# kestrelquantum/QuantumCollocation.jl

Hardware: AMD Instinct MI355X
Metric: full-trajectory constraint+Jacobian evals/s, 3-qubit T=1000 (higher is better)
Workload: dtype f64; 1 GPU; 3-qubit Toffoli UnitarySmoothPulseProblem, T=1000; T=1000 knots (1000/GPU), Pade order 4, free dt; T=1000, N=8, n_drives=6, kernel=mfma, parallelism=knot-shard x1, output_ring_buffers=17

## Files before the change

quantumcollocation.jl_amd/csrc/qc_mfma_exp.hip:

```cpp
#include <stdlib.h>

#include "qc_mfma_common.h"

namespace {

using namespace qc_mfma;

constexpr int kXDeg = 8;
constexpr double kXTh = 0.125;
constexpr int kXMmax = 8;

__device__ inline v4d ximg(const double* __restrict__ Gx, int mat, int lane) {
    const v2d* p = reinterpret_cast<const v2d*>(Gx) + mat * 128 + lane;
    const v2d lo = p[0], hi = p[64];
    return v4d{lo[0], lo[1], hi[0], hi[1]};
}
template <int CTRL>
__device__ inline double xdpp(double x) {
    int lo = __double2loint(x), hi = __double2hiint(x);
    lo = __builtin_amdgcn_update_dpp(0, lo, CTRL, 0xf, 0xf, false);
    hi = __builtin_amdgcn_update_dpp(0, hi, CTRL, 0xf, 0xf, false);
    return __hiloint2double(hi, lo);
}
__device__ inline double xreadlane(double x, int l) {
    return __hiloint2double(__builtin_amdgcn_readlane(__double2hiint(x), l), __builtin_amdgcn_readlane(__double2loint(x), l));
}

template <int M, bool JAC>
__device__ __forceinline__ void horner_step(const v4d& Y, const v4d (&Gj)[M], v4d& R, v4d (&Q)[M], const v4d& cI) {
    v4d accR = cI;
    v4d acc[M];
    const v4d z = {0.0, 0.0, 0.0, 0.0};
    accR = __builtin_amdgcn_mfma_f64_16x16x4f64(Y[0], R[0], accR, 0, 0, 0);
    if constexpr (JAC) {
#pragma unroll
        for (int q = 0; q < M; ++q) acc[q] = __builtin_amdgcn_mfma_f64_16x16x4f64(Gj[q][0], R[0], z, 0, 0, 0);
    }
#pragma unroll
    for (int kk = 1; kk < 4; ++kk) {
        accR = __builtin_amdgcn_mfma_f64_16x16x4f64(Y[kk], R[kk], accR, 0, 0, 0);
        if constexpr (JAC) {
#pragma unroll
            for (int q = 0; q < M; ++q) acc[q] = __builtin_amdgcn_mfma_f64_16x16x4f64(Gj[q][kk], R[kk], acc[q], 0, 0, 0);
        }
    }
    if constexpr (JAC) {
#pragma unroll
        for (int kk = 0; kk < 4; ++kk) {
#pragma unroll
            for (int q = 0; q < M; ++q) acc[q] = __builtin_amdgcn_mfma_f64_16x16x4f64(Y[kk], Q[q][kk], acc[q], 0, 0, 0);
        }
#pragma unroll
        for (int q = 0; q < M; ++q) Q[q] = acc[q];
    }
    R = accR;
}

template <int M>
__device__ __forceinline__ void horner_step_ell(const v4d& Y, const double (&tw)[M][4], const int (&tc)[M][4], double* __restrict__ scr, v4d& R,
                                                v4d (&Q)[M], const v4d& cI, int g, int j) {
#pragma unroll
    for (int r = 0; r < 4; ++r) scr[(4 * r + g) * 17 + j] = R[r];
    __builtin_amdgcn_fence(__ATOMIC_RELEASE, "wavefront");
    __builtin_amdgcn_wave_barrier();
    __builtin_amdgcn_fence(__ATOMIC_ACQUIRE, "wavefront");
    double x[M][4];
#pragma unroll
    for (int q = 0; q < M; ++q) {
#pragma unroll
        for (int r = 0; r < 4; ++r) x[q][r] = scr[tc[q][r]];
    }
    __builtin_amdgcn_sched_barrier(0);
    const v4d z = {0.0, 0.0, 0.0, 0.0};
    v4d accR = cI, acc[M];
#pragma unroll
    for (int kk = 0; kk < 4; ++kk) {
        accR = __builtin_amdgcn_mfma_f64_16x16x4f64(Y[kk], R[kk], accR, 0, 0, 0);
#pragma unroll
        for (int q = 0; q < M; ++q) acc[q] = __builtin_amdgcn_mfma_f64_16x16x4f64(Y[kk], Q[q][kk], kk == 0 ? z : acc[q], 0, 0, 0);
    }
#pragma unroll
    for (int q = 0; q < M; ++q) {
#pragma unroll
        for (int r = 0; r < 4; ++r) Q[q][r] = __builtin_fma(tw[q][r], x[q][r], acc[q][r]);
    }
    R = accR;
    __builtin_amdgcn_fence(__ATOMIC_RELEASE, "wavefront");
    __builtin_amdgcn_wave_barrier();
    __builtin_amdgcn_fence(__ATOMIC_ACQUIRE, "wavefront");
}

template <int M, bool JAC>
__device__ __forceinline__ void square_step(const v4d& Et, const v4d (&Kt)[M], v4d& E, v4d (&L)[M]) {
    const v4d z = {0.0, 0.0, 0.0, 0.0};
    v4d accE = z, acc[M];
#pragma unroll
    for (int kk = 0; kk < 4; ++kk) {
        accE = __builtin_amdgcn_mfma_f64_16x16x4f64(Et[kk], E[kk], accE, 0, 0, 0);
        if constexpr (JAC) {
#pragma unroll
            for (int q = 0; q < M; ++q) acc[q] = __builtin_amdgcn_mfma_f64_16x16x4f64(Et[kk], L[q][kk], kk == 0 ? z : acc[q], 0, 0, 0);
        }
    }
    if constexpr (JAC) {
#pragma unroll
        for (int kk = 0; kk < 4; ++kk) {
#pragma unroll
            for (int q = 0; q < M; ++q) acc[q] = __builtin_amdgcn_mfma_f64_16x16x4f64(Kt[q][kk], E[kk], acc[q], 0, 0, 0);
        }
#pragma unroll
        for (int q = 0; q < M; ++q) L[q] = acc[q];
    }
    E = accE;
}

template <bool JAC, int kMU, int kW, bool ELL = false, int kIPW = 1>
__global__ __launch_bounds__(64 * kW * kIPW, kW) void qc_mfma16_exp_kernel(const QcParams P, const double* __restrict__ Z, double* __restrict__ F,
                                                                    double* __restrict__ J) {
    qc_kernarg_touch<sizeof(QcParams) + 64>();
    static_assert(kIPW == 1 || kW == 2, "two intervals per workgroup: the two-wave forms");
    __shared__ double scr_all[kIPW * kW * (kMU + 1) * 16 * 17];
    const int lane = threadIdx.x & 63;
    const int wq = kIPW * kW > 1 ? __builtin_amdgcn_readfirstlane(threadIdx.x >> 6) : 0;
    const int wv = kW > 1 ? wq % kW : 0;
    double* __restrict__ scr = scr_all + wq * ((kMU + 1) * 16 * 17);
    const int d0 = wv * kMU;
    const int m = P.m;
    const int g = lane >> 4, j = lane & 15, jj = j & 7;
    const bool ft = P.off_dt >= 0;
    const double* __restrict__ Gx = P.Gx;
    const v4d IdB = identity_B(g, j);
    const v4d zero = {0.0, 0.0, 0.0, 0.0};

    {
        const int b = qc_xcd_remap((int)blockIdx.x, (P.n_int + kIPW - 1) / kIPW) * kIPW + wq / kW;
        if (b >= P.n_int) return;
        const long long t = P.t_begin + b;
        const double* __restrict__ z0 = Z + t * (long long)P.zdim;
        const double* __restrict__ z1 = z0 + P.zdim;
        double* __restrict__ Jb = JAC ? J + (size_t)b * P.J_stride + P.J_off : nullptr;
        double* __restrict__ Fb = F ? F + (size_t)b * P.F_stride + P.F_off : nullptr;
        const double h = ft ? z0[P.off_dt] : opaque_scalar(P.dt_fixed);

        const int nc = P.nc, jc = jj < nc ? jj : 0, nr = P.n;
        v4d u0, u1;
#pragma unroll
        for (int r = 0; r < 4; ++r) {
            const int row = 4 * r + g;
            u0[r] = row < nr ? z0[P.off_U + jc * nr + row] : 0.0;
            u1[r] = row < nr ? z1[P.off_U + jc * nr + row] : 0.0;
        }
        v4d Gj[kMU];
        double tw[kMU][4];
        int tc[kMU][4];
        v4d Ga = ximg(Gx, 0, lane);
        {
            constexpr int kMA = kXMmax;
            v4d img[kMA];
            double ak[kMA];
#pragma unroll
            for (int u = 0; u < kMA; ++u) {
                const int k = u < m ? u : (m > 0 ? m - 1 : 0);
                img[u] = ximg(Gx, m > 0 ? k + 1 : 0, lane);
                ak[u] = (u < m) ? z0[P.off_a + k] : 0.0;
            }
            if constexpr (ELL) {
                const double* __restrict__ bw = reinterpret_cast<const double*>(P.ell16);
                const int* __restrict__ bc = reinterpret_cast<const int*>(reinterpret_cast<const char*>(P.ell16) + kXMmax * 32 * 8);
#pragma unroll
                for (int u = 0; u < kMU; ++u) {
#pragma unroll
                    for (int r = 0; r < 4; ++r) {
                        tw[u][r] = bw[(d0 + u) * 32 + 4 * r + g];
                        tc[u][r] = bc[(d0 + u) * 32 + 4 * r + g] * 17 + j;
                    }
                }
            } else {
#pragma unroll
                for (int u = 0; u < kMU; ++u) {
                    const int k = d0 + u;
                    Gj[u] = ximg(Gx, k < m ? k + 1 : 0, lane);
                }
            }
#pragma unroll
            for (int u = 0; u < kMA; ++u) Ga += ak[u] * img[u];
        }
        if constexpr (!ELL) {
#pragma unroll
            for (int u = 0; u < kMU; ++u) if (d0 + u >= m) Gj[u] = zero;
        }

        int sq = 0;
        {
            double best = 0.0;
            bool bad = false;
#pragma unroll
            for (int kk = 0; kk < 4; ++kk) {
                double c = fabs(h * Ga[kk]);
                c += xdpp<0x128>(c);
                c += xdpp<0x124>(c);
                c += xdpp<0x122>(c);
                c += xdpp<0x121>(c);
#pragma unroll
                for (int r = 0; r < 4; ++r) {
                    const double v = xreadlane(c, 16 * r);
                    if (!(v == v) || v > 1e300) bad = true;
                    best = fmax(best, v);
                }
            }
            if (!bad && best > kXTh) {
                int e;
                (void)frexp(best / kXTh, &e);
                sq = e;
                if (ldexp(kXTh, e - 1) >= best) sq = e - 1;
                sq = sq < 0 ? 0 : (sq > 60 ? 60 : sq);
            }
        }
        const double sc = ldexp(1.0, -sq);
        const v4d Y = (h * sc) * Ga;

        double fact = 1.0;
#pragma unroll
        for (int k = 2; k <= kXDeg; ++k) fact *= (double)k;
        double ck = 1.0 / fact;
        v4d R = ck * IdB;
        v4d Q[kMU];
#pragma unroll
        for (int u = 0; u < kMU; ++u) Q[u] = zero;
#pragma unroll 1
        for (int k = kXDeg; k >= 1; --k) {
            ck *= (double)k;
            if constexpr (ELL) horner_step_ell<kMU>(Y, tw, tc, scr, R, Q, ck * IdB, g, j);
            else horner_step<kMU, JAC>(Y, Gj, R, Q, ck * IdB);
        }
        for (int q = 0; q < sq; ++q) {
            v4d Et, Kt[kMU];
            if constexpr (JAC) {
                v4d in[kMU + 1], out[kMU + 1];
                in[0] = R;
#pragma unroll
                for (int u = 0; u < kMU; ++u) in[u + 1] = Q[u];
                lds_transpose16_multi<kMU + 1>(scr, in, out, g, j);
                Et = out[0];
#pragma unroll
                for (int u = 0; u < kMU; ++u) Kt[u] = out[u + 1];
            } else {
                Et = lds_transpose16(scr, R, g, j);
            }
            square_step<kMU, JAC>(Et, Kt, R, Q);
        }
        const v4d Et = lds_transpose16(scr, R, g, j);
        const v4d EU = mm16(Et, u0);
        if (Fb && wv == 0) {
            const v4d dT = lds_transpose16(scr, u1 - EU, g, j);
#pragma unroll
            for (int r = 0; r < 2; ++r) if (4 * r + g < nc && j < nr) qc_st8m<2>(Fb + (4 * r + g) * nr + j, dT[r]);
        }
        if constexpr (JAC) {
            double* pF = Jb + P.jo_F;
            const v4d mE = -Et;
#pragma unroll
            for (int q = wv * (8 / kW); q < (wv + 1) * (8 / kW); ++q) {
                if (q < nc) {
#pragma unroll
                    for (int r = 0; r < 4; ++r) if (4 * r + g < nr && j < nr) qc_st8m<2>(pF + q * nr * nr + (4 * r + g) * nr + j, mE[r]);
                }
            }
            if (wv == kW - 1) for (int i = lane; i < P.s; i += 64) Jb[P.jo_B + i] = 1.0;
            const double fac = -(h * sc);
            v4d Kt[kMU], XT[kMU], ua[kMU];
            lds_transpose16_multi<kMU>(scr, Q, Kt, g, j);
#pragma unroll
            for (int u = 0; u < kMU; ++u) ua[u] = u0;
            mm16_multi<kMU>(ua, Kt, XT);
#pragma unroll
            for (int u = 0; u < kMU; ++u) {
                if (d0 + u < m) {
#pragma unroll
                    for (int r = 0; r < 2; ++r)
                        if (4 * r + g < nc && j < nr) qc_st8m<2>(Jb + P.jo_a + (size_t)(d0 + u) * P.s + (4 * r + g) * nr + j, fac * XT[u][r]);
                }
            }
            if (ft && wv == 0) {
                const v4d GEU = mm16(Ga, EU);
                const v4d hT = lds_transpose16(scr, -GEU, g, j);
#pragma unroll
                for (int r = 0; r < 2; ++r) if (4 * r + g < nc && j < nr) qc_st8m<2>(Jb + P.jo_h + (4 * r + g) * nr + j, hT[r]);
            }
        }
        if (wv == kW - 1) deriv_rows_generic(P, z0, z1, h, Fb, Jb, lane, false);
    }
}

}

bool qc_mfma_exp_supported(const QcParams& P) {
    return P.integrator == QC_EXPONENTIAL && P.n <= 16 && P.nc <= 8 && P.m <= kXMmax;
}

hipError_t qc_launch_mfma_exp(const QcParams& P, bool ell, const double* dZ, double* dF, double* dJ, hipStream_t st) {
    const int grid = P.n_int;
#define QC_XJ1(MU_, W_, I_) do { const int wgs = (grid + I_ - 1) / I_; \
                            if (ell) hipLaunchKernelGGL((qc_mfma16_exp_kernel<true, MU_, W_, true, I_>), dim3(wgs), dim3(64 * W_ * I_), 0, st, P, dZ, dF, dJ); \
                            else hipLaunchKernelGGL((qc_mfma16_exp_kernel<true, MU_, W_, false, I_>), dim3(wgs), dim3(64 * W_ * I_), 0, st, P, dZ, dF, dJ); } while (0)
#define QC_XJ(MU_, W_) do { if (W_ == 2 && grid > 256) QC_XJ1(MU_, W_, (W_ == 2 ? 2 : 1)); else QC_XJ1(MU_, W_, 1); } while (0)
    if (!dJ) {
        hipLaunchKernelGGL((qc_mfma16_exp_kernel<false, 1, 1>), dim3(grid), dim3(64), 0, st, P, dZ, dF, dJ);
    } else if (P.m <= 1) {
        QC_XJ(1, 1);
    } else if (!ell && P.n_int >= 768) {
        if (P.m <= 2) hipLaunchKernelGGL((qc_mfma16_exp_kernel<true, 2, 1>), dim3(grid), dim3(64), 0, st, P, dZ, dF, dJ);
        else if (P.m <= 4) hipLaunchKernelGGL((qc_mfma16_exp_kernel<true, 4, 1>), dim3(grid), dim3(64), 0, st, P, dZ, dF, dJ);
        else if (P.m <= 6) hipLaunchKernelGGL((qc_mfma16_exp_kernel<true, 6, 1>), dim3(grid), dim3(64), 0, st, P, dZ, dF, dJ);
        else hipLaunchKernelGGL((qc_mfma16_exp_kernel<true, 8, 1>), dim3(grid), dim3(64), 0, st, P, dZ, dF, dJ);
    } else {
        const int mh = (P.m + 1) / 2;
        if (mh == 1) QC_XJ(1, 2);
        else if (mh == 2) QC_XJ(2, 2);
        else if (mh == 3) QC_XJ(3, 2);
        else QC_XJ(4, 2);
    }
#undef QC_XJ
#undef QC_XJ1
    return hipGetLastError();
}
```

Measured before the change: 125,000 evals/s (T=1000-equivalent).

## Replace degree-8 Horner Taylor exp with degree-12 Paterson-Stockmeyer evaluation

Replaces the degree-8 Horner Taylor evaluation of the matrix exponential (threshold 1/8) with a degree-12 Taylor polynomial evaluated Paterson–Stockmeyer style from powers A, A², A³, A⁴ plus two outer products, with the scaling threshold raised to 1/2. The aim is fewer MFMA products per interval, both from fewer squarings and from fewer polynomial steps, including the Fréchet-derivative (Jacobian) chains. To do this it parks intermediate sums in extra LDS, adds transposes, and lowers occupancy for kMU>=4 through the launch bounds. That adds LDS pressure and register use, and the larger threshold may change accuracy. Profiling and validation scripts are added alongside.

```diff
diff --git a/profiles/exp_mfma_model.py b/profiles/exp_mfma_model.py
--- /dev/null
+++ b/profiles/exp_mfma_model.py
@@ -0,0 +1,35 @@
+#!/usr/bin/env python3
+import collections
+import math
+import os
+import sys
+
+import numpy as np
+
+sys.path.insert(0, os.path.dirname(os.path.dirname(os.path.abspath(__file__))))
+import __graft_entry__ as g
+
+
+def squarings(norm, th):
+    if not norm > th:
+        return 0
+    e = math.frexp(norm / th)[1]
+    return e - 1 if math.ldexp(th, e - 1) >= norm else e
+
+
+qc = g.load_package()
+inp = qc.config_inputs(3, T=1000, integrator="exponential")
+tr, sys_ = inp.traj, inp.integrators[0].system
+Z = tr.datavec.reshape(tr.T, -1)
+m = sys_.n_drives
+G0, Gd = np.array(sys_.G_drift), np.array(sys_.G_drives).reshape(m, 16, 16)
+a, dt = Z[:, tr.offset("a"):tr.offset("a") + m], Z[:, tr.offset("Δt")]
+norms = [np.abs(dt[t] * (G0 + np.tensordot(a[t], Gd, 1))).sum(axis=0).max() for t in range(tr.T - 1)]
+kW, kMU = 2, 3
+gather, product = 4 + 4 * kMU, 4 + 8 * kMU
+outputs = kW * (4 + 4 * kMU) + 4
+for name, th, fixed in (("degree 8, Horner, threshold 1/8", 0.125, 8 * gather), ("degree 12 in five products, threshold 1/2", 0.5, 3 * gather + 2 * product)):
+    sq = [squarings(x, th) for x in norms]
+    jac = sum(kW * (fixed + s * product) + outputs for s in sq)
+    res = sum((8 if th == 0.125 else 5) * 4 + 4 * s + 4 for s in sq)
+    print(f"{name}: squarings {dict(sorted(collections.Counter(sq).items()))}; F + dF {jac} MFMAs a launch ({jac / len(sq):.1f} an interval), F alone {res}")
diff --git a/profiles/exp_outputs.py b/profiles/exp_outputs.py
--- /dev/null
+++ b/profiles/exp_outputs.py
@@ -0,0 +1,34 @@
+#!/usr/bin/env python3
+import os
+import sys
+
+import numpy as np
+
+ROOT = os.path.dirname(os.path.dirname(os.path.abspath(__file__)))
+sys.path.insert(0, ROOT)
+sys.path.insert(0, os.path.join(ROOT, "tests"))
+
+
+def rel(a, b):
+    return float(np.max(np.abs(a - b) / np.maximum(np.abs(b), 1e-300), initial=0.0, where=b != 0))
+
+
+if sys.argv[1] == "dump":
+    import __graft_entry__ as g
+    import oracle.qc_oracle_c as oc
+    from oracle_bridge import problem_from_inputs
+    qc = g.load_package()
+    inp = qc.config_inputs(3, T=1000, integrator="exponential")
+    dyn = qc.QuantumDynamics(inp.integrators, inp.traj)
+    F, J = dyn.F_dF(inp.traj.datavec, fresh=True)
+    Fa = dyn.F(inp.traj.datavec, fresh=True)
+    Fo, Jo = oc.COracle(problem_from_inputs(inp)).F_dF(inp.traj.datavec)
+    np.savez(sys.argv[2], F=F, J=J)
+    print(f"variant {os.environ.get('QCOLLOC_HIP_VARIANT', 'product')} {dyn.kernel_names[0]}: against the C oracle  F max abs {np.abs(F - Fo).max():.3e}  "
+          f"dF max abs {np.abs(J - Jo).max():.3e} (max |dF| {np.abs(Jo).max():.3f})  F alone == F of F + dF: {np.array_equal(Fa, F)}", flush=True)
+    dyn.close()
+else:
+    A, B = np.load(sys.argv[2]), np.load(sys.argv[3])
+    for k in ("F", "J"):
+        print(f"{k}: largest absolute difference {np.abs(A[k] - B[k]).max():.3e}, largest relative difference (entries above 1e-9) "
+              f"{rel(np.where(np.abs(B[k]) > 1e-9, A[k], 0.0), np.where(np.abs(B[k]) > 1e-9, B[k], 0.0)):.3e}")
diff --git a/profiles/exp_pmc_driver.py b/profiles/exp_pmc_driver.py
--- /dev/null
+++ b/profiles/exp_pmc_driver.py
@@ -0,0 +1,28 @@
+#!/usr/bin/env python3
+import os
+import sys
+
+import numpy as np
+import torch
+
+sys.path.insert(0, os.path.dirname(os.path.dirname(os.path.abspath(__file__))))
+import __graft_entry__ as g
+
+qc = g.load_package()
+inp = qc.config_inputs(3, T=1000, integrator="exponential")
+dyn = qc.QuantumDynamics(inp.integrators, inp.traj)
+d = dyn.dims
+Z = torch.from_numpy(inp.traj.datavec).cuda()
+mu = torch.from_numpy(np.random.default_rng(0).standard_normal(int(d.n_rows))).cuda()
+F = torch.empty(int(d.F_len), dtype=torch.float64, device="cuda")
+J = torch.empty(int(d.jac_nnz), dtype=torch.float64, device="cuda")
+H = torch.empty(int(d.hess_nnz), dtype=torch.float64, device="cuda")
+st = torch.cuda.current_stream()
+jac, res, hes = dyn.bind_F_dF_device(Z, F, J, st), dyn.bind_F_dF_device(Z, F, None, st), dyn.bind_mu_d2F_device(Z, mu, H, st)
+for _ in range(20):
+    jac()
+    res()
+    hes()
+torch.cuda.synchronize()
+print("kernels", dyn.kernel_names, "intervals", int(d.n_intervals))
+dyn.close()
diff --git a/quantumcollocation.jl_amd/csrc/qc_mfma_exp.hip b/quantumcollocation.jl_amd/csrc/qc_mfma_exp.hip
--- a/quantumcollocation.jl_amd/csrc/qc_mfma_exp.hip
+++ b/quantumcollocation.jl_amd/csrc/qc_mfma_exp.hip
@@ -6,8 +6,9 @@
 
 using namespace qc_mfma;
 
-constexpr int kXDeg = 8;
-constexpr double kXTh = 0.125;
+constexpr double kXTh = 0.5;
+constexpr double kXc2 = 1.0 / 2.0, kXc3 = 1.0 / 6.0, kXc4 = 1.0 / 24.0, kXc5 = 1.0 / 120.0, kXc6 = 1.0 / 720.0, kXc7 = 1.0 / 5040.0,
+                 kXc8 = 1.0 / 40320.0, kXc9 = 1.0 / 362880.0, kXc10 = 1.0 / 3628800.0, kXc11 = 1.0 / 39916800.0, kXc12 = 1.0 / 479001600.0;
 constexpr int kXMmax = 8;
 
 __device__ inline v4d ximg(const double* __restrict__ Gx, int mat, int lane) {
@@ -27,7 +28,7 @@
 }
 
 template <int M, bool JAC>
-__device__ __forceinline__ void horner_step(const v4d& Y, const v4d (&Gj)[M], v4d& R, v4d (&Q)[M], const v4d& cI) {
+__device__ __forceinline__ void power_step(const v4d& Y, const v4d (&Gj)[M], v4d& R, v4d (&Q)[M], const v4d& cI) {
     v4d accR = cI;
     v4d acc[M];
     const v4d z = {0.0, 0.0, 0.0, 0.0};
@@ -57,7 +58,7 @@
 }
 
 template <int M>
-__device__ __forceinline__ void horner_step_ell(const v4d& Y, const double (&tw)[M][4], const int (&tc)[M][4], double* __restrict__ scr, v4d& R,
+__device__ __forceinline__ void power_step_ell(const v4d& Y, const double (&tw)[M][4], const int (&tc)[M][4], double* __restrict__ scr, v4d& R,
                                                 v4d (&Q)[M], const v4d& cI, int g, int j) {
 #pragma unroll
     for (int r = 0; r < 4; ++r) scr[(4 * r + g) * 17 + j] = R[r];
@@ -114,16 +115,53 @@
     E = accE;
 }
 
+template <int M, bool JAC>
+__device__ __forceinline__ void outer_step(const v4d& At, const v4d (&Dt)[M], const v4d& X, const v4d (&Xd)[M], v4d& C, v4d (&Cd)[M]) {
+    v4d accC = C, acc[M];
+#pragma unroll
+    for (int kk = 0; kk < 4; ++kk) {
+        accC = __builtin_amdgcn_mfma_f64_16x16x4f64(At[kk], X[kk], accC, 0, 0, 0);
+        if constexpr (JAC) {
+#pragma unroll
+            for (int q = 0; q < M; ++q) acc[q] = __builtin_amdgcn_mfma_f64_16x16x4f64(At[kk], Xd[q][kk], kk == 0 ? Cd[q] : acc[q], 0, 0, 0);
+        }
+    }
+    if constexpr (JAC) {
+#pragma unroll
+        for (int kk = 0; kk < 4; ++kk) {
+#pragma unroll
+            for (int q = 0; q < M; ++q) acc[q] = __builtin_amdgcn_mfma_f64_16x16x4f64(Dt[q][kk], X[kk], acc[q], 0, 0, 0);
+        }
+#pragma unroll
+        for (int q = 0; q < M; ++q) Cd[q] = acc[q];
+    }
+    C = accC;
+}
+
+__device__ __forceinline__ v4d lin3(double a, const v4d& x, double b, const v4d& y, double c, const v4d& z) {
+    v4d o;
+#pragma unroll
+    for (int r = 0; r < 4; ++r) o[r] = __builtin_fma(c, z[r], __builtin_fma(b, y[r], a * x[r]));
+    return o;
+}
+__device__ __forceinline__ v4d axpy(double a, const v4d& x, const v4d& y) {
+    v4d o;
+#pragma unroll
+    for (int r = 0; r < 4; ++r) o[r] = __builtin_fma(a, x[r], y[r]);
+    return o;
+}
 template <bool JAC, int kMU, int kW, bool ELL = false, int kIPW = 1>
-__global__ __launch_bounds__(64 * kW * kIPW, kW) void qc_mfma16_exp_kernel(const QcParams P, const double* __restrict__ Z, double* __restrict__ F,
+__global__ __launch_bounds__(64 * kW * kIPW, kMU >= 4 ? 1 : kW) void qc_mfma16_exp_kernel(const QcParams P, const double* __restrict__ Z, double* __restrict__ F,
                                                                     double* __restrict__ J) {
     qc_kernarg_touch<sizeof(QcParams) + 64>();
     static_assert(kIPW == 1 || kW == 2, "two intervals per workgroup: the two-wave forms");
-    __shared__ double scr_all[kIPW * kW * (kMU + 1) * 16 * 17];
+    constexpr int kScr = (kMU + 1) * (16 * 17 + 256);
+    __shared__ double scr_all[kIPW * kW * kScr];
     const int lane = threadIdx.x & 63;
     const int wq = kIPW * kW > 1 ? __builtin_amdgcn_readfirstlane(threadIdx.x >> 6) : 0;
     const int wv = kW > 1 ? wq % kW : 0;
-    double* __restrict__ scr = scr_all + wq * ((kMU + 1) * 16 * 17);
+    double* __restrict__ scr = scr_all + wq * kScr;
+    double* __restrict__ park = scr + (kMU + 1) * 16 * 17;
     const int d0 = wv * kMU;
     const int m = P.m;
     const int g = lane >> 4, j = lane & 15, jj = j & 7;
@@ -219,19 +257,106 @@
         const double sc = ldexp(1.0, -sq);
         const v4d Y = (h * sc) * Ga;
 
-        double fact = 1.0;
-#pragma unroll
-        for (int k = 2; k <= kXDeg; ++k) fact *= (double)k;
-        double ck = 1.0 / fact;
-        v4d R = ck * IdB;
-        v4d Q[kMU];
-#pragma unroll
-        for (int u = 0; u < kMU; ++u) Q[u] = zero;
-#pragma unroll 1
-        for (int k = kXDeg; k >= 1; --k) {
-            ck *= (double)k;
-            if constexpr (ELL) horner_step_ell<kMU>(Y, tw, tc, scr, R, Q, ck * IdB, g, j);
-            else horner_step<kMU, JAC>(Y, Gj, R, Q, ck * IdB);
+        const auto drive_B = [&](int u) {
+            v4d o;
+#pragma unroll
+            for (int r = 0; r < 4; ++r) o[r] = tc[u][r] == 18 * j ? tw[u][r] : 0.0;
+            return o;
+        };
+        v4d R, Q[kMU];
+        if constexpr (JAC && !ELL) {
+            v4d in[kMU + 1], out[kMU + 1];
+            in[0] = Y;
+#pragma unroll
+            for (int u = 0; u < kMU; ++u) in[u + 1] = Gj[u];
+            lds_transpose16_multi<kMU + 1>(scr, in, out, g, j);
+            R = out[0];
+#pragma unroll
+            for (int u = 0; u < kMU; ++u) Q[u] = out[u + 1];
+        } else {
+            R = lds_transpose16(scr, Y, g, j);
+#pragma unroll
+            for (int u = 0; u < kMU; ++u) {
+                if constexpr (ELL) Q[u] = drive_B(u);
+                else Q[u] = zero;
+            }
+        }
+        __builtin_amdgcn_sched_barrier(0);
+        const auto next_power = [&]() {
+            if constexpr (ELL) power_step_ell<kMU>(Y, tw, tc, scr, R, Q, zero, g, j);
+            else power_step<kMU, JAC>(Y, Gj, R, Q, zero);
+            __builtin_amdgcn_sched_barrier(0);
+        };
+        const v4d P1 = R;
+        v4d D1[ELL ? 1 : kMU];
+        if constexpr (JAC && !ELL) {
+#pragma unroll
+            for (int u = 0; u < kMU; ++u) D1[u] = Q[u];
+        }
+        next_power();
+        const v4d P2 = R;
+        v4d D2[kMU];
+        if constexpr (JAC) {
+#pragma unroll
+            for (int u = 0; u < kMU; ++u) D2[u] = Q[u];
+        }
+        next_power();
+        v4d S1, S2, S1d[kMU], S2d[kMU];
+        {
+            const v4d S0 = lin3(kXc3, R, kXc2, P2, 1.0, IdB + P1);
+#pragma unroll
+            for (int r = 0; r < 4; ++r) park[r * 64 + lane] = S0[r];
+            S1 = lin3(kXc4, IdB, kXc5, P1, 1.0, lin3(kXc6, P2, kXc7, R, 0.0, zero));
+            S2 = lin3(kXc8, IdB, kXc9, P1, 1.0, lin3(kXc10, P2, kXc11, R, 0.0, zero));
+        }
+        if constexpr (JAC) {
+#pragma unroll
+            for (int u = 0; u < kMU; ++u) {
+                v4d d1;
+                if constexpr (ELL) d1 = drive_B(u);
+                else d1 = D1[u];
+                const v4d S0 = lin3(kXc3, Q[u], kXc2, D2[u], 1.0, d1);
+#pragma unroll
+                for (int r = 0; r < 4; ++r) park[(4 * (u + 1) + r) * 64 + lane] = S0[r];
+                S1d[u] = lin3(kXc5, d1, kXc6, D2[u], kXc7, Q[u]);
+                S2d[u] = lin3(kXc9, d1, kXc10, D2[u], kXc11, Q[u]);
+            }
+        }
+        __builtin_amdgcn_sched_barrier(0);
+        next_power();
+        S2 = axpy(kXc12, R, S2);
+        if constexpr (JAC) {
+#pragma unroll
+            for (int u = 0; u < kMU; ++u) S2d[u] = axpy(kXc12, Q[u], S2d[u]);
+        }
+        {
+            v4d At, Dt[kMU];
+            if constexpr (JAC) {
+                v4d in[kMU + 1], out[kMU + 1];
+                in[0] = R;
+#pragma unroll
+                for (int u = 0; u < kMU; ++u) in[u + 1] = Q[u];
+                lds_transpose16_multi<kMU + 1>(scr, in, out, g, j);
+                At = out[0];
+#pragma unroll
+                for (int u = 0; u < kMU; ++u) Dt[u] = out[u + 1];
+            } else {
+                At = lds_transpose16(scr, R, g, j);
+            }
+            __builtin_amdgcn_sched_barrier(0);
+            outer_step<kMU, JAC>(At, Dt, S2, S2d, S1, S1d);
+            __builtin_amdgcn_sched_barrier(0);
+#pragma unroll
+            for (int r = 0; r < 4; ++r) R[r] = park[r * 64 + lane];
+            if constexpr (JAC) {
+#pragma unroll
+                for (int u = 0; u < kMU; ++u) {
+#pragma unroll
+                    for (int r = 0; r < 4; ++r) Q[u][r] = park[(4 * (u + 1) + r) * 64 + lane];
+                }
+            }
+            outer_step<kMU, JAC>(At, Dt, S1, S1d, R, Q);
+            __builtin_amdgcn_sched_barrier(0);
         }
         for (int q = 0; q < sq; ++q) {
             v4d Et, Kt[kMU];
```

Result: no change. 124,600 evals/s (T=1000-equivalent) (-0.3%).
